# AzureLeon1/DiffSpectra

Hardware: AMD Instinct MI355X
Metric: molecules/sec, 1000-step QM9S all-spectra sampling (partial run) (higher is better)
Workload: dtype f32 (GEMMs as split-fp16 x3 MFMA with fp32 accumulate; fp32-level accuracy, parity gates unchanged)

## Files before the change

### diffspectra_amd/csrc/ds_kernels.hip

```cpp
#include <hip/hip_runtime.h>
#include <math.h>
#include <stdint.h>
#include <stdio.h>
#include <stdlib.h>

#include <atomic>
#include <mutex>
#include <utility>
#include <vector>

#include "../../include/diffspectra_hip.h"
#include "ds_device.h"
#include "ds_train_common.h"

#define ADAC DS_ADA_COLS
constexpr int DS_NODE_PF = 8;
constexpr int DS_NODE_PF2 = 4;
constexpr int DS_QKV_PF = 4;
constexpr int DS_TWO_STREAM_MAX_PAIRS = 400000;

#ifdef DS_STAMPS
#define DS_STAMP_INIT()                                                                                 \
  unsigned long long _sa[16] = {0, 0, 0, 0, 0, 0, 0, 0, 0, 0, 0, 0, 0, 0, 0, 0};                        \
  unsigned long long _t0 = __builtin_amdgcn_s_memtime()
#define DS_STAMP(i)                                                                                     \
  do {                                                                                                  \
    const unsigned long long _t1 = __builtin_amdgcn_s_memtime();                                        \
    _sa[i] += _t1 - _t0;                                                                                \
    _t0 = _t1;                                                                                          \
  } while (0)
#define DS_STAMP_W(i)                                                                                   \
  do {                                                                                                  \
    asm volatile("s_waitcnt vmcnt(0) lgkmcnt(0)" ::: "memory");                                         \
    DS_STAMP(i);                                                                                        \
  } while (0)
#define DS_STAMP_FLUSH(t)                                                                               \
  do {                                                                                                  \
    if (threadIdx.x == (t))                                                                             \
      for (int _i = 0; _i < 16; ++_i)                                                                   \
        if (_sa[_i]) atomicAdd(reinterpret_cast<unsigned long long*>(c.ws.flags + 16) + _i, _sa[_i]);   \
  } while (0)
#else
#define DS_STAMP_INIT()
#define DS_STAMP(i)
#define DS_STAMP_W(i)
#define DS_STAMP_FLUSH(t)
#endif

namespace {

struct Ctx {
  ds_layout L;
  ds_workspace ws;
  const float* wbase;
  const int64_t* woff;
  float edge_th, cutoff;
};

__device__ __forceinline__ const float* BW(const Ctx& c, int blk, int slot) {
  return c.wbase + c.woff[blk * DS_W_BLOCK_SLOTS + slot];
}
__device__ __forceinline__ const float* GW(const Ctx& c, int slot) {
  return c.wbase + c.woff[DS_NBLOCKS * DS_W_BLOCK_SLOTS + slot];
}

__device__ __forceinline__ float rbf_feature(float x, int k, const float* __restrict__ mean, const float* __restrict__ stdv,
                                             const float* __restrict__ astd) {
  if (k == 0) return x;
  const float z = (x - mean[k - 1]) / stdv[k - 1];
  return expf(-0.5f * (z * z)) / astd[k - 1];
}

__global__ void k_time_feat(Ctx c, const float* __restrict__ noise_level) {
  const int b = blockIdx.x * blockDim.x + threadIdx.x;
  if (b >= c.L.B) return;
  const float* w = GW(c, DS_GW_SIN_W);
  const float x = noise_level[b];
  float* f = c.ws.tfeat + (size_t)b * 24;
  f[0] = x;
  for (int i = 0; i < 8; ++i) {
    const float fr = ((x * w[i]) * 2.0f) * 3.14159265358979323846f;
    f[1 + i] = sinf(fr);
    f[9 + i] = cosf(fr);
  }
  for (int i = 17; i < 24; ++i) f[i] = 0.0f;
}

__global__ void k_pair_flags(Ctx c, const float* __restrict__ cond_x, const float* __restrict__ cond_edge_x) {
  const int p = blockIdx.x * blockDim.x + threadIdx.x;
  const bool valid = p < c.L.Pp;
  int bits = 3;
  bool nonzero = false;
  if (valid && cond_x != nullptr) {
    const int da = c.L.node_dense[c.L.pair_a[p]], db = c.L.node_dense[c.L.pair_b[p]];
    const float* pa = cond_x + (size_t)da * 9;
    const float* pb = cond_x + (size_t)db * 9;
    const float dx = pa[0] - pb[0], dy = pa[1] - pb[1], dz = pa[2] - pb[2];
    const float d2 = dx * dx + dy * dy + dz * dz;
    const int m = c.L.pair_mol[p];
    const int lb = db - m * c.L.N;
    const float ce = cond_edge_x[((size_t)da * c.L.N + lb) * 2 + 0];
    bits = (ce >= c.edge_th ? 1 : 0) | (d2 <= c.cutoff ? 2 : 0);
    nonzero = d2 != 0.0f;
  }
  if (valid) c.ws.adj[p] = bits;
  if (cond_x != nullptr) {
    const int any = __syncthreads_or(nonzero ? 1 : 0);
    if (any && threadIdx.x == 0) __hip_atomic_store(&c.ws.flags[0], 1, __ATOMIC_RELAXED, __HIP_MEMORY_SCOPE_AGENT);
  }
}

__global__ __launch_bounds__(256) void k_node_init(Ctx c, const float* __restrict__ xh, const float* __restrict__ cond_x) {
  constexpr int R = 8;
  const int row0 = blockIdx.x * R;
  const int col = threadIdx.x;
  __shared__ __attribute__((aligned(16))) float in[R][16];
  if (col < R * 16) {
    const int rr = col >> 4, k = col & 15, row = row0 + rr;
    float v = 0.0f;
    if (row < c.L.Nn) {
      const int d = c.L.node_dense[row];
      if (k < 6) v = xh[(size_t)d * 9 + 3 + k];
      else if (k < 12) v = cond_x ? cond_x[(size_t)d * 9 + 3 + (k - 6)] : 0.0f;
      else if (k < 15) v = xh[(size_t)d * 9 + (k - 12)];
    }
    in[rr][k] = v;
  }
  __syncthreads();
  const float* W = GW(c, DS_GW_NODE_EMB_W);
  float w[12];
#pragma unroll
  for (int k = 0; k < 12; ++k) w[k] = wp_at(W, 256, k, col);
  const float bias = GW(c, DS_GW_NODE_EMB_B)[col];
#pragma unroll
  for (int rr = 0; rr < R; ++rr) {
    const int row = row0 + rr;
    if (row >= c.L.Nn) break;
    float acc = 0.0f;
#pragma unroll
// ... 132 lines not shown
    for (int i = 0; i < 16; ++i) acc[0][i] = bcol;
    acc_zero<1>(lo);
    wave_mma_h_deep<1, false, 8, 8>(&Xh[mt * 32][0], 128, wse, ring, 0, acc, lo);
    split_finish<1>(acc, lo);
#pragma unroll
    for (int i = 0; i < 16; ++i) Y[mt * 32 + acc_row(i, lane >> 5)][cc * 32 + (lane & 31)] = acc[0][i];
  }
  __syncthreads();
  {
    const int lane = tid & 63, wv = tid >> 6;
    _Float16* ye = reinterpret_cast<_Float16*>(c.ws.ye);
#pragma unroll
    for (int j = 0; j < 4; ++j) {
      const int row = 16 * wv + 4 * j + (lane >> 4);
      const float4 v = ln_mod_reg64(reinterpret_cast<const float4*>(&Y[row][0])[lane & 15], lsh[j], lsc[j]);
      if (row0 + row < c.L.Pp) split_store4(ye + (size_t)(row0 + row) * 128, 64, 4 * (lane & 15), v);
    }
  }
}

template <int NW>
__global__ __launch_bounds__(NW * 64) void k_node_qkv(Ctx c, int blk) {
  ds_fp16_saturate();
  constexpr int NT = NW * 64;
  constexpr int T = 64;
  constexpr int LDH = 2 * 256 + 8;
  __shared__ __attribute__((aligned(16))) _Float16 Xh[T][LDH];
  __shared__ int rmol[T];
  const int tid = threadIdx.x, row0 = blockIdx.x * T, col0 = blockIdx.y * 384;
  if (tid < T) rmol[tid] = (row0 + tid < c.L.Nn) ? c.L.node_mol[row0 + tid] : 0;
  __syncthreads();
  {
    const float* adn = c.ws.ada + blk * DS_ADA_BLOCK_STRIDE + DS_ADA_NODE;
    const int lane = tid & 63, wv = tid >> 6, g = lane >> 4, j = lane & 15;
    static_assert(NT == 256, "four waves x 16 rows");
#pragma unroll
    for (int half = 0; half < 2; ++half) {
      float4 v[2][4], sh[2][4], sc[2][4];
#pragma unroll
      for (int ps = 0; ps < 2; ++ps) {
        const int row = 16 * wv + 8 * half + 4 * ps + g;
        const float4* hp = reinterpret_cast<const float4*>(c.ws.h + (size_t)min(row0 + row, c.L.Nn - 1) * 256) + j;
        const float4* ap = reinterpret_cast<const float4*>(adn + (size_t)rmol[row] * ADAC) + j;
#pragma unroll
        for (int u = 0; u < 4; ++u) {
          v[ps][u] = hp[16 * u];
          sh[ps][u] = ap[16 * u];
          sc[ps][u] = ap[64 + 16 * u];
        }
      }
#pragma unroll
      for (int ps = 0; ps < 2; ++ps) {
        const int row = 16 * wv + 8 * half + 4 * ps + g;
        ln_mod_quad256(v[ps], sh[ps], sc[ps]);
#pragma unroll
        for (int u = 0; u < 4; ++u)
          split_store4(&Xh[row][0], 256, 64 * u + 4 * j, row0 + row < c.L.Nn ? v[ps][u] : make_float4(0, 0, 0, 0));
      }
    }
  }
  __syncthreads();
  const float* bias = BW(c, blk, DS_BW_QKV_B) + col0;
  float* qkv = c.ws.qkv + (size_t)row0 * 768 + col0;
  const int valid = c.L.Nn - row0, wave = tid >> 6;
  for (int ch = wave; ch < 12; ch += NW) {
    asm volatile("" ::: "memory");
    const float b = bias[ch * 32 + (tid & 31)];
    f32x16 acc[2], lo[2];
#pragma unroll
    for (int m = 0; m < 2; ++m)
#pragma unroll
      for (int i = 0; i < 16; ++i) acc[m][i] = b;
    acc_zero<2>(lo);
    wave_mma_h_ring<2, false, 16, DS_QKV_PF>(&Xh[0][0], 256, BW(c, blk, DS_BW_QKV_H), 768, 256, col0 + ch * 32, 0, acc, lo);
    split_finish<2>(acc, lo);
    acc_store<2, 768>(acc, qkv + ch * 32, valid, [](int, float v) { return v; });
  }
}

__global__ __launch_bounds__(1024) void k_attn_fused(Ctx c, int blk) {
  ds_fp16_saturate();
  DS_STAMP_INIT();
  constexpr int NT = 1024, QS = 512 + 32, LDT = 256 + 4, LDY = 2 * 64 + 8, CR = 32, MAXP = DS_MAX_ATOMS * (DS_MAX_ATOMS - 1) / 2;
  __shared__ __attribute__((aligned(16))) float QK[DS_MAX_ATOMS * QS];
  __shared__ __attribute__((aligned(16))) float Tt[2][CR][LDT];
  __shared__ __attribute__((aligned(16))) _Float16 Yc[2][CR][LDY];
  __shared__ __attribute__((aligned(16))) float AL[2][CR][32];
  __shared__ int PT[(MAXP + 15) & ~15];
  __shared__ int VT[32][32];
  static_assert(DS_MAX_ATOMS <= 32 && MAXP <= 511 - CR, "visit table packing");
  static_assert(DS_MAX_ATOMS * 128 <= 4 * NT && DS_MAX_ATOMS * 64 <= 2 * NT && MAXP <= NT, "single-pass staging");
  const int tid = threadIdx.x, wave = tid >> 6, lane = tid & 63, hh = lane >> 5;
  int n0, n, p0, P;
  if (c.L.mol_by_size) {
    const int4 r = reinterpret_cast<const int4*>(c.L.mol_by_size)[blockIdx.x];
    n0 = r.x; n = r.y; p0 = r.z; P = r.w;
  } else {
    const int m = blockIdx.x;
    n0 = c.L.node_off[m]; n = c.L.node_off[m + 1] - n0;
    p0 = c.L.pair_off[m]; P = c.L.pair_off[m + 1] - p0;
  }
  const WStreamH ws_e0 = wstream_h(BW(c, blk, DS_BW_E0_H), 256, 64, (wave & 7) * 32);
  const WStreamH ws_e1 = wstream_h(BW(c, blk, DS_BW_E1_H), 256, 64, (wave & 7) * 32);
  if (n <= 0) return;
  if (P <= 0) {
    for (int i = tid; i < 256; i += NT) c.ws.attn[(size_t)n0 * 256 + i] = 0.0f;
    return;
  }
  const int nch = (P + CR - 1) / CR;
  const bool producer = wave >= 8;
  const int ptid = tid & 511, prow = ptid >> 4, ppiece = ptid & 15;
  const u32x4* ye4 = reinterpret_cast<const u32x4*>(c.ws.ye) + (size_t)p0 * 16;
  auto row_pair = [&](int R) {
    const int d = R / n + 1, i = R - (d - 1) * n;
    int j = i + d;
    if (j >= n) j -= n;
    const int a = min(i, j), b = max(i, j);
    return a * (2 * n - a - 1) / 2 + (b - a - 1);
  };
  auto fetch_y = [&](int ck, bool class_order) {
    const int R = ck * CR + prow;
    const int Rc = min(R, P - 1);
    return ye4[(size_t)(class_order ? PT[Rc] : Rc) * 16 + ppiece];
  };
  auto commit_y = [&](int buf, const u32x4& v) { *reinterpret_cast<u32x4*>(&Yc[buf][prow][ppiece * 8]) = v; };
  h8 wf[2][4];
  auto load_weights = [&](const WStreamH& ws_) {
#pragma unroll
    for (int pl = 0; pl < 2; ++pl)
#pragma unroll
      for (int kb = 0; kb < 4; ++kb) wf[pl][kb] = wload_h(ws_, pl, kb);
  };
  auto project = [&](int buf) {
    f32x16 acc[1], lo[1];
    acc_zero<1>(acc);
    acc_zero<1>(lo);
    const _Float16* xr = &Yc[buf][lane & 31][8 * hh];
#pragma unroll
    for (int kb = 0; kb < 4; ++kb) {
      const h8 x1 = *reinterpret_cast<const h8*>(xr + kb * 16);
      const h8 x2 = *reinterpret_cast<const h8*>(xr + 64 + kb * 16);
      acc[0] = __builtin_amdgcn_mfma_f32_32x32x16_f16(wf[0][kb], x1, acc[0], 0, 0, 0);
      lo[0] = __builtin_amdgcn_mfma_f32_32x32x16_f16(wf[0][kb], x2, lo[0], 0, 0, 0);
      lo[0] = __builtin_amdgcn_mfma_f32_32x32x16_f16(wf[1][kb], x1, lo[0], 0, 0, 0);
    }
    split_finish<1>(acc, lo);
    float* trow = &Tt[buf][lane & 31][(wave & 7) * 32 + 4 * hh];
#pragma unroll
    for (int q = 0; q < 4; ++q) {
      f32x2 v0, v1;
      v0.x = acc[0][4 * q]; v0.y = acc[0][4 * q + 1]; v1.x = acc[0][4 * q + 2]; v1.y = acc[0][4 * q + 3];
      v0 = ds_tanh2_prescaled(v0); v1 = ds_tanh2_prescaled(v1);
      *reinterpret_cast<float4*>(trow + 8 * q) = make_float4(v0.x, v0.y, v1.x, v1.y);
    }
  };
  auto produce = [&](u32x4 ya, u32x4 yb, bool class_order, auto&& after_first) {
    project(0);
    after_first();
    if (1 < nch) commit_y(1, ya);
    if (3 < nch) ya = fetch_y(3, class_order);
    __syncthreads();
    if (class_order) { DS_STAMP(13); } else { DS_STAMP(9); }
    auto interval = [&](int k, u32x4& B) {
      if (k + 2 < nch) commit_y(k & 1, B);
      if (k + 4 < nch) B = fetch_y(k + 4, class_order);
      if (k + 1 < nch) project((k + 1) & 1);
      if (class_order) { DS_STAMP(14); } else { DS_STAMP(10); }
      __syncthreads();
      if (class_order) { DS_STAMP(15); } else { DS_STAMP(11); }
    };
    for (int k = 0; k < nch; k += 2) {
      interval(k, yb);
      if (k + 1 >= nch) break;
      interval(k + 1, ya);
    }
  };

  {
    u32x4 y0 = {0, 0, 0, 0}, y1 = y0, y2 = y0;
    if (producer) {
      load_weights(ws_e0);
      y0 = fetch_y(0, false);
      y1 = fetch_y(1, false);
      y2 = fetch_y(2, false);
    } else if (tid < P) {
      PT[tid] = ((c.L.pair_a[p0 + tid] - n0) << 8) | (c.L.pair_b[p0 + tid] - n0) | (c.ws.adj[p0 + tid] << 16);
    }
    f32x4 v[4];
#pragma unroll
    for (int u = 0; u < 4; ++u) {
      const int idx = min(tid + u * NT, n * 128 - 1);
      v[u] = reinterpret_cast<const f32x4*>(c.ws.qkv + (size_t)(n0 + (idx >> 7)) * 768)[idx & 127];
    }
    __builtin_amdgcn_sched_barrier(0);
    auto store_qk = [&]() {
      f32x4* junk = reinterpret_cast<f32x4*>(&Tt[1][0][0]) + tid;
#pragma unroll
      for (int u = 0; u < 4; ++u) {
        const int idx = tid + u * NT;
        f32x4* dst = idx < n * 128 ? reinterpret_cast<f32x4*>(QK) + (idx >> 7) * (QS / 4) + (idx & 127) : junk;
        *dst = v[u];
      }
    };
    if (producer) commit_y(0, y0);
    __syncthreads();
    if (producer) { DS_STAMP(8); } else { DS_STAMP(0); }
    if (producer) {
      produce(y1, y2, false, store_qk);
      load_weights(ws_e1);
    } else {
      store_qk();
      __syncthreads();
      DS_STAMP(1);
      const int row = tid >> 4, hs = tid & 15;
      for (int k = 0; k < nch; ++k) {
        const int pl = k * CR + row;
        if (pl < P) {
          const int e_ = PT[pl];
          float* out = c.ws.lg + (size_t)(p0 + pl) * 32;
          if (hs == 14) {
            const float h0 = (e_ & 0x10000) ? 1.0f : -1e10f, h1 = (e_ & 0x20000) ? 1.0f : -1e10f;
            out[0] = h0; out[1] = h1; out[16] = h0; out[17] = h1;
          } else if (hs < 14) {
            const int a = (e_ >> 8) & 255, b = e_ & 255;
            typedef const volatile f32x2 __attribute__((address_space(3))) * lds_v2;
            lds_v2 t0 = (lds_v2)(&Tt[k & 1][row][hs * 18]);
            lds_v2 qa = (lds_v2)(QK + a * QS + hs * 18);
            lds_v2 qb = (lds_v2)(QK + b * QS + hs * 18);
            lds_v2 ka = (lds_v2)(QK + a * QS + 256 + hs * 18);
            lds_v2 kb = (lds_v2)(QK + b * QS + 256 + hs * 18);
            float s_ab = 0.0f, s_ba = 0.0f;
#pragma unroll
            for (int j0 = 0; j0 < 9; j0 += 3) {
              f32x2 e[3], xa[3], xb[3], ya[3], yb[3];
#pragma unroll
              for (int j = 0; j < 3; ++j) { e[j] = t0[j0 + j]; xa[j] = qa[j0 + j]; xb[j] = qb[j0 + j]; ya[j] = ka[j0 + j]; yb[j] = kb[j0 + j]; }
#pragma unroll
              for (int j = 0; j < 3; ++j) {
                s_ab = __builtin_fmaf(xb[j].x * ya[j].x, e[j].x, s_ab); s_ab = __builtin_fmaf(xb[j].y * ya[j].y, e[j].y, s_ab);
                s_ba = __builtin_fmaf(xa[j].x * yb[j].x, e[j].x, s_ba); s_ba = __builtin_fmaf(xa[j].y * yb[j].y, e[j].y, s_ba);
              }
            }
            out[2 + hs] = s_ab / 4.0f;
            out[16 + 2 + hs] = s_ba / 4.0f;
          }
        }
        DS_STAMP(2);
        __syncthreads();
        DS_STAMP(3);
      }
    }
  }
  __threadfence_block();
  __syncthreads();
  float* V = QK;
  int* ET = reinterpret_cast<int*>(&Tt[0][0][0]);
  {
    const int t = tid >> 5, q = tid & 31, d = (q >> 1) + 1;
    int e = 511;
    if (t < n && q < n - 1) {
      int i, s_;
      if (2 * d == n) {
        i = t < d ? t : t - d;
        s_ = t < d ? t + d : t - d;
      } else {
        int sa = t + d, ib = t - d;
        if (sa >= n) sa -= n;
        if (ib < 0) ib += n;
        const bool first_is_a = t < ib;
        const bool take_a = (q & 1) ? !first_is_a : first_is_a;
        i = take_a ? t : ib;
        s_ = take_a ? sa : ib;
      }
      e = ((d - 1) * n + i) | (s_ << 9) | ((s_ < t ? 0 : 1) << 14);
    }
    VT[t][q] = e;
    const int s = q;
    int eo = -1;
    if (t < n && s < n && s != t) {
      const int lo_ = s < t ? s : t, hi_ = s < t ? t : s;
      eo = (lo_ * (2 * n - lo_ - 1) / 2 + (hi_ - lo_ - 1)) * 32 + (s < t ? 0 : 16);
    }
    ET[t * 32 + s] = eo;
    if (tid < P) PT[tid] = row_pair(tid);
  }
  f32x4 vst[2];
#pragma unroll
  for (int u = 0; u < 2; ++u) {
    const int i0 = min(tid + u * NT, n * 64 - 1);
    vst[u] = reinterpret_cast<const f32x4*>(c.ws.qkv + (size_t)(n0 + (i0 >> 6)) * 768 + 512)[i0 & 63];
  }
  __builtin_amdgcn_sched_barrier(0);
  __syncthreads();
  u32x4 y0 = {0, 0, 0, 0}, y1 = y0, y2 = y0;
  if (producer) {
    y0 = fetch_y(0, true);
    y1 = fetch_y(1, true);
    y2 = fetch_y(2, true);
  }
  auto store_v = [&]() {
    f32x4* junk = reinterpret_cast<f32x4*>(&Yc[0][0][0]) + tid;
#pragma unroll
    for (int u = 0; u < 2; ++u) {
      f32x4* dst = tid + u * NT < n * 64 ? reinterpret_cast<f32x4*>(V) + tid + u * NT : junk;
      *dst = vst[u];
    }
  };
  {
    const int h = lane & 15, sq = (lane >> 4) & 1, t = 2 * wave + hh;
    const int* et = ET + t * 32 + sq;
    float* lgm = c.ws.lg + (size_t)p0 * 32 + h;
    if (t < n) {
      float x[15];
      int eos[15];
      float mx = -INFINITY;
#pragma unroll
      for (int j = 0; j < 15; ++j) eos[j] = et[2 * j];
#pragma unroll
      for (int j = 0; j < 15; ++j) x[j] = lgm[max(eos[j], 0)];
      __builtin_amdgcn_sched_barrier(0);
#pragma unroll
      for (int j = 0; j < 15; ++j) x[j] = eos[j] >= 0 ? x[j] : -INFINITY;
#pragma unroll
      for (int j = 0; j < 15; ++j) mx = fmaxf(mx, x[j]);
      mx = fmaxf(mx, __shfl_xor(mx, 16, 64));
      float sum = 0.0f;
#pragma unroll
      for (int j = 0; j < 15; ++j) {
        x[j] = __expf(x[j] - mx);
        sum += x[j];
      }
      sum += __shfl_xor(sum, 16, 64);
      const float den = sum + 1e-16f;
#pragma unroll
      for (int j = 0; j < 15; ++j)
        if (eos[j] >= 0) lgm[eos[j]] = x[j] / den;
    }
  }
  store_v();
  __threadfence_block();
  __syncthreads();
  if (producer) { DS_STAMP(12); } else { DS_STAMP(4); }
  if (producer) {
    commit_y(0, y0);
    __syncthreads();
    produce(y1, y2, true, [] {});
    DS_STAMP_FLUSH(512);
  } else {
    const int arow = (tid & 255) >> 3, apiece = tid & 7;
    auto fetch_a = [&](int ck) {
      const int R = ck * CR + arow;
      return reinterpret_cast<const u32x4*>(c.ws.lg + (size_t)(p0 + PT[min(R, P - 1)]) * 32)[apiece];
    };
    auto commit_a = [&](int buf, const u32x4& v) {
      if (tid < 256) reinterpret_cast<u32x4*>(&AL[buf][arow][0])[apiece] = v;
    };
    const u32x4 a0 = fetch_a(0);
    u32x4 ab = fetch_a(1), aa = fetch_a(2);
    commit_a(0, a0);
    __syncthreads();
    __syncthreads();
    DS_STAMP(5);
    const int t_me = tid >> 4, q16 = tid & 15;
    const int* vt_row = &VT[t_me][0];
    int vt_q = 0, vt_e = vt_row[0];
    float4 acc[4];
#pragma unroll
    for (int u = 0; u < 4; ++u) acc[u] = make_float4(0, 0, 0, 0);
    auto interval = [&](int k, u32x4& A) {
      if (k + 1 < nch) commit_a((k + 1) & 1, A);
      if (k + 3 < nch) A = fetch_a(k + 3);
      const int R0 = k * CR;
      while ((vt_e & 511) - R0 < CR) {
        const int r = (vt_e & 511) - R0, s_ = (vt_e >> 9) & 31;
        const float4* gp = reinterpret_cast<const float4*>(&Tt[k & 1][r][4 * q16]);
        const float4* vp = reinterpret_cast<const float4*>(V + s_ * 256 + 4 * q16);
        const float* ap = &AL[k & 1][r][((vt_e >> 14) & 1) * 16 + (q16 >> 2)];
        float4 g[4], v[4];
        float al[4];
#pragma unroll
        for (int u = 0; u < 4; ++u) { g[u] = gp[16 * u]; v[u] = vp[16 * u]; al[u] = ap[4 * u]; }
        vt_e = vt_row[++vt_q];
#pragma unroll
        for (int u = 0; u < 4; ++u) {
          acc[u].x += (v[u].x * g[u].x) * al[u]; acc[u].y += (v[u].y * g[u].y) * al[u];
          acc[u].z += (v[u].z * g[u].z) * al[u]; acc[u].w += (v[u].w * g[u].w) * al[u];
        }
      }
      DS_STAMP(6);
      __syncthreads();
      DS_STAMP(7);
    };
    for (int k = 0; k < nch; k += 2) {
      interval(k, ab);
      if (k + 1 >= nch) break;
      interval(k + 1, aa);
    }
    if (t_me < n) {
      float4* o = reinterpret_cast<float4*>(c.ws.attn + (size_t)(n0 + t_me) * 256 + 4 * q16);
#pragma unroll
      for (int u = 0; u < 4; ++u) o[16 * u] = acc[u];
    }
    DS_STAMP_FLUSH(0);
  }
}

__global__ __launch_bounds__(256) void k_node_n2e(Ctx c, int blk) {
  ds_fp16_saturate();
  constexpr int T = 64, LDH = 2 * 256 + 8;
  __shared__ __attribute__((aligned(16))) _Float16 A1[T][LDH];
  const int tid = threadIdx.x, wave = tid >> 6, lane = tid & 63, row0 = blockIdx.x * T;
  const int Nn = c.L.Nn;
  {
    float4 v[16];
#pragma unroll
    for (int u = 0; u < 16; ++u) {
      const int idx = tid + u * 256, row = idx >> 6, k4 = idx & 63;
      v[u] = reinterpret_cast<const float4*>(c.ws.attn + (size_t)min(row0 + row, Nn - 1) * 256)[k4];
    }
#pragma unroll
    for (int u = 0; u < 16; ++u) {
      const int idx = tid + u * 256, row = idx >> 6, k4 = idx & 63;
      split_store4(&A1[row][0], 256, 4 * k4, row0 + row < Nn ? v[u] : make_float4(0, 0, 0, 0));
    }
  }
  __syncthreads();
  const int mt = wave >> 1, cc = wave & 1;
  if (row0 + mt * 32 >= Nn) return;
  f32x16 acc[1], lo[1];
  acc_zero<1>(acc);
  acc_zero<1>(lo);
  wave_mma_h_ring<1, false, 16, DS_NODE_PF>(&A1[mt * 32][0], 256, BW(c, blk, DS_BW_N2E_H), 64, 256, cc * 32, 0, acc, lo);
  split_finish<1>(acc, lo);
  acc_store<1, 64>(acc, c.ws.u + (size_t)(row0 + mt * 32) * 64 + cc * 32, Nn - row0 - mt * 32, [](int, float v) { return v; });
  (void)lane;
}

template <bool N2E>
__global__ __launch_bounds__(256, 2) void k_node_update(Ctx c, int blk) {
  ds_fp16_saturate();
  constexpr int T = 32, LDH = 2 * 256 + 8;
  __shared__ __attribute__((aligned(16))) _Float16 B1[T][LDH];
  __shared__ __attribute__((aligned(16))) _Float16 H2[T][LDH];
  __shared__ int rmol[T];
  const int tid = threadIdx.x, wave = tid >> 6, row0 = blockIdx.x * T;
  const int Nn = c.L.Nn;
  const float* ada = c.ws.ada;
  if (tid < T) rmol[tid] = (row0 + tid < Nn) ? c.L.node_mol[row0 + tid] : 0;
  __syncthreads();
  {
    const int lane = tid & 63, g = lane >> 4, j = lane & 15;
    float4 va[2][4], vh[2][4], vg[2][4], sh[2][4], sc[2][4];
#pragma unroll
    for (int ps = 0; ps < 2; ++ps) {
      const int row = 8 * wave + 4 * ps + g;
      const size_t gr = (size_t)min(row0 + row, Nn - 1);
      const float4* ad = reinterpret_cast<const float4*>(ada + (size_t)rmol[row] * ADAC + blk * DS_ADA_BLOCK_STRIDE + DS_ADA_NODE) + j;
      const float4* ap = reinterpret_cast<const float4*>(c.ws.attn + gr * 256) + j;
      const float4* hp = reinterpret_cast<const float4*>(c.ws.h + gr * 256) + j;
#pragma unroll
      for (int u = 0; u < 4; ++u) {
        va[ps][u] = ap[16 * u];
        vh[ps][u] = hp[16 * u];
        vg[ps][u] = ad[128 + 16 * u];
        sh[ps][u] = ad[192 + 16 * u];
        sc[ps][u] = ad[256 + 16 * u];
      }
    }
#pragma unroll
    for (int ps = 0; ps < 2; ++ps) {
      const int row = 8 * wave + 4 * ps + g;
      float4 r[4];
#pragma unroll
      for (int u = 0; u < 4; ++u) {
        if (row0 + row >= Nn) va[ps][u] = vh[ps][u] = make_float4(0, 0, 0, 0);
        if (N2E) split_store4(&B1[row][0], 256, 64 * u + 4 * j, va[ps][u]);
        r[u].x = vh[ps][u].x + vg[ps][u].x * va[ps][u].x; r[u].y = vh[ps][u].y + vg[ps][u].y * va[ps][u].y;
        r[u].z = vh[ps][u].z + vg[ps][u].z * va[ps][u].z; r[u].w = vh[ps][u].w + vg[ps][u].w * va[ps][u].w;
      }
      ln_mod_quad256(r, sh[ps], sc[ps]);
#pragma unroll
      for (int u = 0; u < 4; ++u) split_store4(&H2[row][0], 256, 64 * u + 4 * j, r[u]);
    }
  }
  __syncthreads();
  if (N2E) {
    if (wave < 2) {
// ... 1168 lines not shown
        if (c_bond2[ta][tb] != 0 && d < (float)(c_bond2[ta][tb] + 5)) {
          order = 2;
          if (c_bond3[ta][tb] != 0 && d < (float)(c_bond3[ta][tb] + 3)) order = 3;
        }
      }
      bonds += order;
      if (bond_order) bond_order[(size_t)dn[a] * N + (dn[b] - m * N)] = order;
    }
    ok = bonds == c_valence[ta] ? 1 : 0;
  }
  const int cnt = __popcll(__ballot(ok != 0));
  if (a == 0) { nr_stable[m] = cnt; mol_stable[m] = cnt == n ? 1 : 0; }
}

__global__ __launch_bounds__(1024) void k_spec_attention(const float* __restrict__ qkv, float* __restrict__ scores,
                                                       float* __restrict__ out, int B, int L, int heads, float scale,
                                                       int has_prev) {
  constexpr int DK = 8;
  extern __shared__ __attribute__((aligned(16))) float kv[];
  const int b = blockIdx.z, h = blockIdx.y, q0 = blockIdx.x * blockDim.x, tid = threadIdx.x;
  const int D = heads * DK;
  float* Ks = kv;
  float* Vs = kv + (size_t)L * DK;
  for (int idx = tid; idx < L * DK; idx += blockDim.x) {
    const int j = idx / DK, d = idx - j * DK;
    const float* base = qkv + ((size_t)b * L + j) * 3 * D + h * DK + d;
    Ks[idx] = base[D];
    Vs[idx] = base[2 * D];
  }
  __syncthreads();
  const int i = q0 + tid;
  if (i >= L) return;
  float q[DK];
  for (int d = 0; d < DK; ++d) q[d] = qkv[((size_t)b * L + i) * 3 * D + h * DK + d];
  float* scol = scores + ((size_t)b * heads + h) * L * L + i;
  float mx = -INFINITY, den = 0.0f, o[DK];
  for (int d = 0; d < DK; ++d) o[d] = 0.0f;
  for (int j0 = 0; j0 < L; j0 += 8) {
    float sv[8];
    float bm = -INFINITY;
#pragma unroll
    for (int u = 0; u < 8; ++u) {
      const int j = min(j0 + u, L - 1);
      float s = 0.0f;
#pragma unroll
      for (int d = 0; d < DK; ++d) s += q[d] * Ks[j * DK + d];
      s *= scale;
      if (has_prev) s += scol[(size_t)j * L];
      sv[u] = s;
      if (j0 + u < L) { scol[(size_t)j * L] = s; bm = fmaxf(bm, s); }
    }
    const float nm = fmaxf(mx, bm), r = expf(mx - nm);
    den *= r;
#pragma unroll
    for (int d = 0; d < DK; ++d) o[d] *= r;
#pragma unroll
    for (int u = 0; u < 8; ++u) {
      if (j0 + u < L) {
        const float p = expf(sv[u] - nm);
        den += p;
#pragma unroll
        for (int d = 0; d < DK; ++d) o[d] += p * Vs[(j0 + u) * DK + d];
      }
    }
    mx = nm;
  }
  for (int d = 0; d < DK; ++d) out[((size_t)b * L + i) * D + h * DK + d] = o[d] / den;
}

__global__ void k_layernorm_affine(const float* __restrict__ x, const float* __restrict__ g, const float* __restrict__ bt,
                                   float* __restrict__ y, int rows, int cols, float eps) {
  const int row = blockIdx.x, lane = threadIdx.x;
  if (row >= rows) return;
  const float* xr = x + (size_t)row * cols;
  float s = 0.0f;
  for (int k = lane; k < cols; k += 64) s += xr[k];
  const float mean = wave_sum(s) / (float)cols;
  float v = 0.0f;
  for (int k = lane; k < cols; k += 64) { const float d = xr[k] - mean; v += d * d; }
  const float rstd = 1.0f / sqrtf(wave_sum(v) / (float)cols + eps);
  for (int k = lane; k < cols; k += 64) y[(size_t)row * cols + k] = (xr[k] - mean) * rstd * g[k] + bt[k];
}

bool make_ctx(Ctx& c, const ds_weights* w, const ds_layout* L, const ds_workspace* ws) {
  if (!w || !L || !ws || !w->base || !w->off_dev) return false;
  if (L->max_n > DS_MAX_ATOMS || L->B <= 0) return false;
  c.L = *L; c.ws = *ws; c.wbase = w->base; c.woff = w->off_dev;
  c.edge_th = w->edge_th; c.cutoff = w->spatial_cut_off;
  return true;
}

inline bool layout_ok(const ds_layout* L) { return L && L->B > 0 && L->max_n <= DS_MAX_ATOMS && L->max_n <= L->N; }

inline bool clear(void* p, size_t bytes, hipStream_t s) { return hipMemsetAsync(p, 0, bytes, s) == hipSuccess; }
inline bool record(hipEvent_t ev, hipStream_t s) { return hipEventRecord(ev, s) == hipSuccess; }
inline bool wait(hipStream_t s, hipEvent_t ev) { return hipStreamWaitEvent(s, ev, 0) == hipSuccess; }
constexpr int MAX_DEVICES = 16;

inline int device_cus() {
  static std::atomic<int> cus[MAX_DEVICES];
  int dev = 0, n = 0;
  if (hipGetDevice(&dev) != hipSuccess || dev < 0 || dev >= MAX_DEVICES) return 256;
  if ((n = cus[dev].load(std::memory_order_relaxed)) > 0) return n;
  if (hipDeviceGetAttribute(&n, hipDeviceAttributeMultiprocessorCount, dev) != hipSuccess || n <= 0) n = 256;
  cus[dev].store(n, std::memory_order_relaxed);
  return n;
}

template <int ACT>
__global__ __launch_bounds__(256, 2) void k_gemm_big(GemmArgs g) {
  constexpr int T = 128, KC = 64, LD = KC + DS_LDP;
  __shared__ __attribute__((aligned(16))) float X[2][T][LD];
  const int tid = threadIdx.x, wave = tid >> 6;
  const int row0 = blockIdx.x * T;
  const int col0 = (blockIdx.y * 4 + wave) * 32;
  const bool active = col0 < g.Npad;
  const int nchunks = g.K / KC;
  float4 st[8];
  auto fetch = [&](int kc) {
#pragma unroll
    for (int u = 0; u < 8; ++u) {
      const int idx = tid + u * 256, row = idx >> 4, k4 = idx & 15;
      const size_t gr = (size_t)min(row0 + row, g.M - 1);
      st[u] = reinterpret_cast<const float4*>(g.A + gr * g.lda + (size_t)kc * KC)[k4];
    }
  };
  auto stash = [&](int buf) {
#pragma unroll
    for (int u = 0; u < 8; ++u) {
      const int idx = tid + u * 256, row = idx >> 4, k4 = idx & 15;
      float4 v = st[u];
      if (g.a_silu) { v.x = ds_silu(v.x); v.y = ds_silu(v.y); v.z = ds_silu(v.z); v.w = ds_silu(v.w); }
      if (row0 + row >= g.M) v = make_float4(0, 0, 0, 0);
      reinterpret_cast<float4*>(&X[buf][row][0])[k4] = v;
    }
  };
  f32x16 acc[4];
  acc_zero<4>(acc);
  fetch(0);
  stash(0);
  BFrag bf = bfrag_load(g.Wp, g.Npad, active ? col0 : 0, 0, 8);
  __syncthreads();
  for (int kc = 0; kc < nchunks; ++kc) {
    const int cur = kc & 1;
    if (kc + 1 < nchunks) fetch(kc + 1);
    const float* wp = g.Wp + (size_t)(kc * (KC / 8)) * 2 * g.Npad * 4;
    if (active) wave_mma<4>(&X[cur][0][0], LD, wp, g.Npad, col0, 0, KC / 8, acc, 0, &bf);
    if (kc + 1 < nchunks) {
      stash(cur ^ 1);
      bf = bfrag_load(wp + (size_t)(KC / 8) * 2 * g.Npad * 4, g.Npad, active ? col0 : 0, 0, 8);
    }
    __syncthreads();
  }
  if (!active) return;
  {
    const int lane = tid & 63, r = lane & 31, hh = lane >> 5, col = col0 + r;
    const bool colok = col < g.N;
    const float bcol = (g.bias && colok) ? g.bias[col] : 0.0f;
    const float csc = (g.cs && colok) ? g.cs[col] : 1.0f, csh = (g.cs && colok) ? g.csh[col] : 0.0f;
    const unsigned long long pw = reinterpret_cast<unsigned long long>(g.C + (size_t)row0 * g.ldc + col0);
    const unsigned long long pu = (static_cast<unsigned long long>(__builtin_amdgcn_readfirstlane(static_cast<int>(pw >> 32))) << 32) |
                                  static_cast<unsigned int>(__builtin_amdgcn_readfirstlane(static_cast<int>(pw)));
    const __amdgpu_buffer_rsrc_t rc = __builtin_amdgcn_make_buffer_rsrc(reinterpret_cast<float*>(pu), 0, 0x7fffffff, 0x00020000);
    const int voff = (4 * hh * g.ldc + r) * 4, rowb = g.ldc * 4;
#pragma unroll
    for (int m = 0; m < 4; ++m)
#pragma unroll
      for (int i = 0; i < 16; ++i) {
        const int row = m * 32 + (i & 3) + 8 * (i >> 2), gr = row0 + row + 4 * hh;
        if (gr < g.M && colok) {
          float v = ds_act<ACT>(acc[m][i] + bcol);
// ... 137 lines not shown
  Ctx c;
  if (!make_ctx(c, w, L, ws) || !xh || !edge_x || ((cond_x == nullptr) != (cond_edge_x == nullptr))) return DS_ERR_ARG;
  if (!clear(ws->flags, 8 * sizeof(int32_t), s)) return DS_ERR_LAUNCH;
  if (L->Pp > 0) hipLaunchKernelGGL(k_pair_flags, dim3((L->Pp + 1023) / 1024), dim3(1024), 0, s, c, cond_x, cond_edge_x);
  hipLaunchKernelGGL(k_node_init, dim3((L->Nn + 7) / 8), dim3(256), 0, s, c, xh, cond_x);
  if (L->Pp > 0) hipLaunchKernelGGL(k_pair_init, dim3((L->Pp + 63) / 64), dim3(256), 0, s, c, edge_x, cond_x, cond_edge_x);
  return DST_CHECK_LAUNCH();
}

int ds_stage_block(const ds_weights* w, const ds_layout* L, ds_workspace* ws, int blk, int last, void* stream) {
  hipStream_t s = (hipStream_t)stream;
  Ctx c;
  if (!make_ctx(c, w, L, ws) || blk < 0 || blk >= DS_NBLOCKS) return DS_ERR_ARG;
  launch_edge_geom(c, blk, s);
  launch_node_qkv(c, blk, s);
  launch_attn(c, blk, s);
  launch_node_update<true>(c, blk, s);
  launch_edge_update(c, blk, s);
  launch_equi_pairs(c, blk, s);
  launch_pos_update(c, last, s);
  return DST_CHECK_LAUNCH();
}

int ds_stage_readout(const ds_weights* w, const ds_layout* L, ds_workspace* ws, float* out_xh, float* out_edge, void* stream) {
  hipStream_t s = (hipStream_t)stream;
  Ctx c;
  if (!make_ctx(c, w, L, ws) || !out_xh || !out_edge) return DS_ERR_ARG;
  const size_t nx = (size_t)L->B * L->N * 9, ne = (size_t)L->B * L->N * L->N * 2;
  if (!clear(out_xh, nx * sizeof(float), s) || !clear(out_edge, ne * sizeof(float), s)) return DS_ERR_LAUNCH;
  hipLaunchKernelGGL(k_node_readout, dim3((L->Nn + 31) / 32), dim3(256), 0, s, c, out_xh);
  if (L->Pp > 0) hipLaunchKernelGGL(k_edge_readout, dim3((L->Pp + 127) / 128), dim3(256), 0, s, c, out_edge);
  hipLaunchKernelGGL(k_final_pos, dim3((L->B + 63) / 64), dim3(64), 0, s, c, out_xh);
  return DST_CHECK_LAUNCH();
}

struct SideStream {
  hipStream_t s = nullptr;
  hipEvent_t fork[DS_NBLOCKS + 1] = {}, join[DS_NBLOCKS + 1] = {};
  std::once_flag once;
  bool ok = false;
};
static SideStream g_side[MAX_DEVICES];
static int g_two_stream = -1;

static SideStream* side_stream() {
  int dev = 0;
  if (hipGetDevice(&dev) != hipSuccess || dev < 0 || dev >= MAX_DEVICES) return nullptr;
  SideStream& ss = g_side[dev];
  std::call_once(ss.once, [&ss] {
    bool ok = hipStreamCreateWithFlags(&ss.s, hipStreamNonBlocking) == hipSuccess;
    for (int i = 0; ok && i <= DS_NBLOCKS; ++i)
      ok = hipEventCreateWithFlags(&ss.fork[i], hipEventDisableTiming) == hipSuccess &&
           hipEventCreateWithFlags(&ss.join[i], hipEventDisableTiming) == hipSuccess;
    ss.ok = ok;
  });
  return ss.ok ? &ss : nullptr;
}

static int forward_blocks_two_streams(const ds_weights* w, const ds_layout* L, ds_workspace* ws, hipStream_t s, SideStream* ss) {
  Ctx c;
  if (!make_ctx(c, w, L, ws)) return DS_ERR_ARG;
  hipStream_t s2 = ss->s;
  const hipEvent_t fork0 = ss->fork[DS_NBLOCKS], join0 = ss->join[DS_NBLOCKS];
  if (!record(fork0, s) || !wait(s2, fork0)) return DS_ERR_LAUNCH;
  launch_node_qkv(c, 0, s2);
  if (!record(join0, s2)) return DS_ERR_LAUNCH;
  for (int blk = 0; blk < DS_NBLOCKS; ++blk) {
    launch_edge_geom(c, blk, s);
    if (!wait(s, blk == 0 ? join0 : ss->join[blk - 1])) return DS_ERR_LAUNCH;
    launch_attn(c, blk, s);
    launch_node_n2e(c, blk, s);
    if (!record(ss->fork[blk], s) || !wait(s2, ss->fork[blk])) return DS_ERR_LAUNCH;
    launch_node_update<false>(c, blk, s2);
    if (blk + 1 < DS_NBLOCKS) launch_node_qkv(c, blk + 1, s2);
    if (!record(ss->join[blk], s2)) return DS_ERR_LAUNCH;
    launch_edge_update(c, blk, s);
    if (!wait(s, ss->join[blk])) return DS_ERR_LAUNCH;
    launch_equi_pairs(c, blk, s);
    launch_pos_update(c, blk == DS_NBLOCKS - 1 ? 1 : 0, s);
  }
  return DST_CHECK_LAUNCH();
}

int ds_set_two_stream(int on) {
  const int prev = g_two_stream;
  g_two_stream = on;
  return prev;
}

int ds_forward(const ds_weights* w, const ds_layout* L, ds_workspace* ws, const float* xh, const float* edge_x,
               const float* cond_x, const float* cond_edge_x, const float* noise_level, const float* ctx_emb, float* out_xh,
               float* out_edge, void* stream) {
  int st = ds_stage_time(w, L, ws, noise_level, ctx_emb, stream);
  if (st) return st;
  st = ds_stage_init(w, L, ws, xh, edge_x, cond_x, cond_edge_x, stream);
  if (st) return st;
  static const int env_two = [] { const char* e = getenv("DIFFSPECTRA_TWO_STREAM"); return e ? atoi(e) : -1; }();
  const int pick = g_two_stream >= 0 ? g_two_stream : env_two;
  const int two = pick >= 0 ? pick : (L->Pp < DS_TWO_STREAM_MAX_PAIRS ? 1 : 0);
  SideStream* ss = two ? side_stream() : nullptr;
  if (ss) {
    st = forward_blocks_two_streams(w, L, ws, (hipStream_t)stream, ss);
    if (st) return st;
  } else {
    for (int b = 0; b < DS_NBLOCKS; ++b) {
      st = ds_stage_block(w, L, ws, b, b == DS_NBLOCKS - 1, stream);
      if (st) return st;
    }
  }
  return ds_stage_readout(w, L, ws, out_xh, out_edge, stream);
}

int ds_sampler_step(const ds_layout* L, float c_x, float c_pred, float sigma, float temperature, float* x, float* edge_x,
                     const float* pred, const float* edge_pred, const float* raw_pos, const float* raw_feat,
                     const float* raw_edge, float* x_mean, float* edge_mean, void* stream) {
  if (!layout_ok(L) || !x || !edge_x || !pred || !edge_pred || !raw_pos || !raw_feat || !raw_edge || !x_mean || !edge_mean) return DS_ERR_ARG;
  hipLaunchKernelGGL(k_sampler_step, dim3(L->B), dim3(256), 0, (hipStream_t)stream, *L, c_x, c_pred, sigma, temperature, x,
                     edge_x, pred, edge_pred, raw_pos, raw_feat, raw_edge, x_mean, edge_mean);
  return DST_CHECK_LAUNCH();
}

int ds_initial_noise(const ds_layout* L, uint64_t seed, const int64_t* mol_id, float* x, float* edge_x, void* stream) {
  if (!layout_ok(L) || !mol_id || !x || !edge_x) return DS_ERR_ARG;
  hipStream_t s = (hipStream_t)stream;
  const size_t nb = (size_t)L->B * L->N;
  if (!clear(x, nb * 9 * sizeof(float), s) || !clear(edge_x, nb * L->N * 2 * sizeof(float), s)) return DS_ERR_LAUNCH;
  hipLaunchKernelGGL(k_noise_step<0>, dim3(L->B), dim3(256), 0, s, *L, 0.0f, 0.0f, 0.0f, 0.0f, (unsigned long long)seed, 0u, mol_id,
                     x, edge_x, (const float*)nullptr, (const float*)nullptr, (float*)nullptr, (float*)nullptr,
                     (const float*)nullptr, (const int32_t*)nullptr);
  return DST_CHECK_LAUNCH();
}

int ds_sampler_step_philox(const ds_layout* L, float c_x, float c_pred, float sigma, float temperature, uint64_t seed, int32_t step,
                           const int64_t* mol_id, float* x, float* edge_x, const float* pred, const float* edge_pred,
                           float* x_mean, float* edge_mean, void* stream) {
  if (!layout_ok(L) || !mol_id || !x || !edge_x || !pred || !edge_pred || !x_mean || !edge_mean || step < 0) return DS_ERR_ARG;
  hipLaunchKernelGGL(k_noise_step<1>, dim3(L->B), dim3(256), 0, (hipStream_t)stream, *L, c_x, c_pred, sigma, temperature,
                     (unsigned long long)seed, (unsigned int)step + 1u, mol_id, x, edge_x, pred, edge_pred, x_mean, edge_mean,
                     (const float*)nullptr, (const int32_t*)nullptr);
  return DST_CHECK_LAUNCH();
}

int ds_step_begin(const float* table, int32_t n_steps, int32_t* step, int32_t B, float* noise_level, void* stream) {
  if (!table || !step || !noise_level || B <= 0 || n_steps <= 0) return DS_ERR_ARG;
  hipLaunchKernelGGL(k_step_begin, dim3(1), dim3(256), 0, (hipStream_t)stream, table, n_steps, step, B, noise_level);
  return DST_CHECK_LAUNCH();
}

int ds_sampler_step_philox_dev(const ds_layout* L, const float* table, const int32_t* step, float temperature, uint64_t seed,
                               const int64_t* mol_id, float* x, float* edge_x, const float* pred, const float* edge_pred,
                               float* x_mean, float* edge_mean, void* stream) {
  if (!layout_ok(L) || !table || !step || !mol_id || !x || !edge_x || !pred || !edge_pred || !x_mean || !edge_mean) return DS_ERR_ARG;
  hipLaunchKernelGGL(k_noise_step<2>, dim3(L->B), dim3(256), 0, (hipStream_t)stream, *L, 0.0f, 0.0f, 0.0f, temperature,
                     (unsigned long long)seed, 0u, mol_id, x, edge_x, pred, edge_pred, x_mean, edge_mean, table, step);
  return DST_CHECK_LAUNCH();
}

int ds_post_process(const ds_layout* L, const float* xh, const float* edge_x, float* pos_out, int32_t* atom_type, int32_t* fc,
                    float* edge_type, void* stream) {
  if (!layout_ok(L) || !xh || !edge_x || !pos_out || !atom_type || !fc || !edge_type) return DS_ERR_ARG;
  hipStream_t s = (hipStream_t)stream;
  const size_t nb = (size_t)L->B * L->N;
  if (!clear(pos_out, nb * 3 * sizeof(float), s) || !clear(atom_type, nb * sizeof(int32_t), s) || !clear(fc, nb * sizeof(int32_t), s) ||
      !clear(edge_type, nb * L->N * sizeof(float), s))
    return DS_ERR_LAUNCH;
  hipLaunchKernelGGL(k_post_process, dim3(L->B), dim3(128), 0, s, *L, xh, edge_x, pos_out, atom_type, fc, edge_type);
// ... 58 lines not shown
```

### include/diffspectra_hip.h

```cpp
#ifndef DIFFSPECTRA_HIP_H
#define DIFFSPECTRA_HIP_H

#include <stdint.h>

#ifdef __cplusplus
extern "C" {
#endif

#define DS_OK 0
#define DS_ERR_ARG (-1)
#define DS_ERR_LAUNCH (-2)

#define DS_NBLOCKS 8
#define DS_HID 256
#define DS_EHID 64
#define DS_TDIM 1024
#define DS_ADA_BLOCK_STRIDE 2464
#define DS_ADA_NODE 0
#define DS_ADA_EDGE 1536
#define DS_ADA_EQUI 1920
#define DS_ADA_DIST 2432
#define DS_ADA_TOP (DS_NBLOCKS * DS_ADA_BLOCK_STRIDE)
#define DS_ADA_COLS (DS_ADA_TOP + 32)

// ... 40 lines not shown
};
#define DS_W_NUM_SLOTS (DS_NBLOCKS * DS_W_BLOCK_SLOTS + DS_W_GLOBAL_SLOTS)

#define DS_MAX_ATOMS 29
#define DS_RECORD_BYTES 1248
#define DS_REC_POS 0
#define DS_REC_TYPE (DS_MAX_ATOMS * 12)
#define DS_REC_FC (DS_REC_TYPE + DS_MAX_ATOMS)
#define DS_REC_BOND (DS_REC_FC + DS_MAX_ATOMS)
#define DS_REC_BOND_END (DS_REC_BOND + DS_MAX_ATOMS * DS_MAX_ATOMS)
#ifdef __cplusplus
static_assert(DS_REC_BOND_END <= DS_RECORD_BYTES && DS_RECORD_BYTES % 4 == 0, "a record holds its fields and is a whole number of dwords");
static_assert((DS_REC_BOND_END + 3) / 4 * 4 <= DS_RECORD_BYTES, "the dwords that cover the bond block stay inside the record");
#endif


typedef struct ds_weights {
  const float* base;
  const int64_t* off_dev;
  int64_t off[DS_W_NUM_SLOTS];
  float edge_th;
  float spatial_cut_off;
} ds_weights;

typedef struct ds_layout {
  int32_t B, N, Nn, Pp;
  int32_t max_n;
  int32_t _pad;
  const int32_t* node_off;
  const int32_t* pair_off;
  const int32_t* node_dense;
  const int32_t* node_mol;
  const int32_t* pair_a;
  const int32_t* pair_b;
  const int32_t* pair_mol;
  const int32_t* mol_by_size;
} ds_layout;

typedef struct ds_workspace {
  float* pos;
  float* h;
  float* e;
  float* atom_hids;
  float* edge_hids;
  float* tfeat;
  float* tmid;
  float* temb_silu;
  float* ada;
  float* qkv;
  float* ye;
  float* dist;
  float* attn;
  float* u;
  float* ac;
  float* ed;
  float* lg;
  float* tr;
  int32_t* adj;
  int32_t* flags;
} ds_workspace;

void ds_struct_sizes(int64_t* out);

typedef struct ds_gemm_args {
  const float* A; int64_t lda; int32_t a_grp_rows; int32_t _p0; int64_t a_grp_stride;
  const float* Wp; const float* bias;
  float* C; int64_t ldc; int32_t c_grp_rows; int32_t _p1; int64_t c_grp_stride;
  int32_t M, K, N, act;
  const float* R; int64_t ldr; int32_t r_grp_rows; int32_t a_silu;
  const float* col_scale; const float* col_shift;
} ds_gemm_args;
int ds_gemm(const ds_gemm_args* args, void* stream);

int ds_gemm_split(const void* A_split, const float* W_split, const float* bias, float* C, int64_t ldc, int32_t M, int32_t K,
                  int32_t N, void* stream);

int ds_forward(const ds_weights* w, const ds_layout* L, ds_workspace* ws,
               const float* xh, const float* edge_x, const float* cond_x, const float* cond_edge_x,
               const float* noise_level, const float* ctx_emb,
               float* out_xh, float* out_edge, void* stream);

int ds_set_two_stream(int on);

int ds_stage_time(const ds_weights* w, const ds_layout* L, ds_workspace* ws, const float* noise_level,
                  const float* ctx_emb, void* stream);
int ds_stage_init(const ds_weights* w, const ds_layout* L, ds_workspace* ws, const float* xh, const float* edge_x,
                  const float* cond_x, const float* cond_edge_x, void* stream);
int ds_stage_block(const ds_weights* w, const ds_layout* L, ds_workspace* ws, int block, int last, void* stream);
int ds_stage_readout(const ds_weights* w, const ds_layout* L, ds_workspace* ws, float* out_xh, float* out_edge,
                     void* stream);

int ds_sampler_step(const ds_layout* L, float c_x, float c_pred, float sigma, float temperature,
                    float* x, float* edge_x, const float* pred, const float* edge_pred,
                    const float* raw_pos, const float* raw_feat, const float* raw_edge,
                    float* x_mean, float* edge_mean, void* stream);

int ds_initial_noise(const ds_layout* L, uint64_t seed, const int64_t* mol_id, float* x, float* edge_x, void* stream);
int ds_sampler_step_philox(const ds_layout* L, float c_x, float c_pred, float sigma, float temperature,
                           uint64_t seed, int32_t step, const int64_t* mol_id,
                           float* x, float* edge_x, const float* pred, const float* edge_pred,
                           float* x_mean, float* edge_mean, void* stream);

int ds_step_begin(const float* table, int32_t n_steps, int32_t* step, int32_t B, float* noise_level, void* stream);
int ds_sampler_step_philox_dev(const ds_layout* L, const float* table, const int32_t* step, float temperature,
                               uint64_t seed, const int64_t* mol_id, float* x, float* edge_x, const float* pred,
                               const float* edge_pred, float* x_mean, float* edge_mean, void* stream);

int ds_post_process(const ds_layout* L, const float* xh, const float* edge_x,
                    float* pos_out, int32_t* atom_type, int32_t* fc, float* edge_type, void* stream);

int ds_check_stability(const ds_layout* L, const float* pos, const int32_t* atom_type, int32_t* bond_order,
                       int32_t* nr_stable, int32_t* mol_stable, void* stream);

int ds_match_records(const uint8_t* prb_rec, const int32_t* prb_n, int64_t P, const uint8_t* ref_rec, const int32_t* ref_n, int64_t M,
                     const int64_t* ref_index, float max_distance, int32_t min_atoms, double* rmsd, int32_t* n_matched,
                     float* type_acc, float* bond_acc, uint8_t* exact, int32_t* map, void* stream);

#define DS_GRAPH_DIFFERENT 0
#define DS_GRAPH_IDENTICAL 1
#define DS_GRAPH_UNDECIDED 2
#define DS_GRAPH_INVALID 3
#define DS_GRAPH_MAX_NODES 1048576
int ds_graph_identity_records(const uint8_t* prb_rec, const int32_t* prb_n, int64_t P, const uint8_t* ref_rec, const int32_t* ref_n, int64_t M,
                              const int64_t* ref_index, int32_t max_nodes, uint8_t* verdict, int32_t* nodes, int32_t* map, void* stream);

int ds_graph_hash_records(const uint8_t* rec, const int32_t* n, int64_t P, uint64_t* hash, void* stream);

#define DS_MCES_EXACT 0
#define DS_MCES_UNDECIDED 2
#define DS_MCES_INVALID 3
#define DS_MCES_MAX_NODES 4194304
int ds_mces_records(const uint8_t* prb_rec, const int32_t* prb_n, int64_t P, const uint8_t* ref_rec, const int32_t* ref_n, int64_t M,
                    const int64_t* ref_index, int32_t drop_h, int32_t max_nodes, int32_t* dist, int32_t* lower, uint8_t* status,
                    int32_t* nodes, int32_t* map, void* stream);

#define DS_MORGAN_MAX_RADIUS 3
#define DS_MORGAN_MAX_FEATURES 116
#define DS_MORGAN_MAX_BITS 4096
#define DS_MORGAN_OK 0
#define DS_MORGAN_INVALID 3
int ds_morgan_records(const uint8_t* rec, const int32_t* n, int64_t P, int32_t drop_h, int32_t radius, uint64_t* ids, int32_t* count,
                      void* stream);
int ds_morgan_similarity_records(const uint8_t* prb_rec, const int32_t* prb_n, int64_t P, const uint8_t* ref_rec, const int32_t* ref_n, int64_t M,
                                 const int64_t* ref_index, int32_t drop_h, int32_t radius, int32_t n_bits, int32_t* common, int32_t* n_prb,
                                 int32_t* n_ref, uint8_t* status, void* stream);

#define DS_GEOM_MAX_CLASSES 32
int ds_geometry_count_records(const uint8_t* rec, const int32_t* n, int64_t P, const int32_t* bond_cls, int32_t n_bond_cls,
                              const int32_t* angle_cls, int32_t n_angle_cls, const int32_t* dihedral_cls, int32_t n_dihedral_cls,
                              int32_t* counts, int32_t* skipped, void* stream);
int ds_geometry_fill_records(const uint8_t* rec, const int32_t* n, int64_t P, const int32_t* bond_cls, int32_t n_bond_cls,
                             const int32_t* angle_cls, int32_t n_angle_cls, const int32_t* dihedral_cls, int32_t n_dihedral_cls,
                             int64_t total_bond, int64_t total_angle, int64_t total_dihedral, const int64_t* offsets,
                             float* bond_value, uint8_t* bond_class, float* angle_value, uint8_t* angle_class,
                             float* dihedral_value, uint8_t* dihedral_class, void* stream);

#define DS_MMD_TILE 256
#define DS_MMD_CHUNKS 128
#define DS_MMD_MAX_SAMPLES 1048576
#define DS_MMD_MAX_KERNELS 8
#define DS_MMD_MAX_CLASSES 65535
#define DS_MMD_OK 0
#define DS_MMD_EMPTY 1
#define DS_MMD_INVALID 2
int ds_mmd_1d_workspace_bytes(int64_t n_classes, int64_t* bytes);
int ds_mmd_1d_segments(const float* x, const int64_t* x_off, int64_t Nx, const float* y, const int64_t* y_off, int64_t Ny, int64_t n_classes,
// ... 18 lines not shown
```

Before: 232.5.

## Keep attention logits and weights in LDS arena instead of global round-trip

The fused attention kernel now carves a single LDS arena of about 160KB. When a molecule's q|k tile and per-pair logits fit, the logits and softmax weights stay in shared memory instead of round-tripping through the global lg buffer. That removes the global fetch/commit pipeline for alpha tiles and the block-scope fences. The visit table gains a packed pair index so the aggregation step can read alpha from LDS directly, and global lg is still written for later consumers. The larger LDS footprint may reduce occupancy, and there is an env/API toggle.

```diff
diff --git a/diffspectra_amd/csrc/ds_kernels.hip b/diffspectra_amd/csrc/ds_kernels.hip
--- a/diffspectra_amd/csrc/ds_kernels.hip
+++ b/diffspectra_amd/csrc/ds_kernels.hip
@@ -6,6 +6,7 @@
 
 #include <atomic>
 #include <mutex>
+#include <type_traits>
 #include <utility>
 #include <vector>
 
@@ -55,6 +56,7 @@
   const float* wbase;
   const int64_t* woff;
   float edge_th, cutoff;
+  int attn_lds;
 };
 
 __device__ __forceinline__ const float* BW(const Ctx& c, int blk, int slot) {
@@ -353,13 +355,15 @@
   ds_fp16_saturate();
   DS_STAMP_INIT();
   constexpr int NT = 1024, QS = 512 + 32, LDT = 256 + 4, LDY = 2 * 64 + 8, CR = 32, MAXP = DS_MAX_ATOMS * (DS_MAX_ATOMS - 1) / 2;
-  __shared__ __attribute__((aligned(16))) float QK[DS_MAX_ATOMS * QS];
   __shared__ __attribute__((aligned(16))) float Tt[2][CR][LDT];
   __shared__ __attribute__((aligned(16))) _Float16 Yc[2][CR][LDY];
-  __shared__ __attribute__((aligned(16))) float AL[2][CR][32];
   __shared__ int PT[(MAXP + 15) & ~15];
   __shared__ int VT[32][32];
-  static_assert(DS_MAX_ATOMS <= 32 && MAXP <= 511 - CR, "visit table packing");
+  constexpr int QK_F = DS_MAX_ATOMS * QS, AL_F = 2 * CR * 32;
+  constexpr int ARENA_F = (160 * 1024 - (int)(sizeof(Tt) + sizeof(Yc) + sizeof(PT) + sizeof(VT))) / 4 & ~3;
+  __shared__ __attribute__((aligned(16))) float ARENA[ARENA_F];
+  static_assert(QK_F + AL_F <= ARENA_F && QK_F % 4 == 0, "the global path's q|k and alpha tiles");
+  static_assert(DS_MAX_ATOMS <= 32 && MAXP <= 511 - CR && MAXP <= (1 << 16), "visit table packing: row 9 bits, source 5, direction 1, pair row 16");
   static_assert(DS_MAX_ATOMS * 128 <= 4 * NT && DS_MAX_ATOMS * 64 <= 2 * NT && MAXP <= NT, "single-pass staging");
   const int tid = threadIdx.x, wave = tid >> 6, lane = tid & 63, hh = lane >> 5;
   int n0, n, p0, P;
@@ -378,6 +382,12 @@
     for (int i = tid; i < 256; i += NT) c.ws.attn[(size_t)n0 * 256 + i] = 0.0f;
     return;
   }
+  const bool lds_lg = c.attn_lds && n * QS + P * 32 <= ARENA_F;
+  float* const QK = ARENA;
+  float (*const AL)[CR][32] = reinterpret_cast<float (*)[CR][32]>(ARENA + QK_F);
+  float* const LG = ARENA + ARENA_F - P * 32;
+  auto body = [&](auto lds_tag) {
+  constexpr bool LDS_LG = decltype(lds_tag)::value;
   const int nch = (P + CR - 1) / CR;
   const bool producer = wave >= 8;
   const int ptid = tid & 511, prow = ptid >> 4, ppiece = ptid & 15;
@@ -488,7 +498,7 @@
         const int pl = k * CR + row;
         if (pl < P) {
           const int e_ = PT[pl];
-          float* out = c.ws.lg + (size_t)(p0 + pl) * 32;
+          float* out = LDS_LG ? LG + pl * 32 : c.ws.lg + (size_t)(p0 + pl) * 32;
           if (hs == 14) {
             const float h0 = (e_ & 0x10000) ? 1.0f : -1e10f, h1 = (e_ & 0x20000) ? 1.0f : -1e10f;
             out[0] = h0; out[1] = h1; out[16] = h0; out[17] = h1;
@@ -522,7 +532,7 @@
       }
     }
   }
-  __threadfence_block();
+  if constexpr (!LDS_LG) __threadfence_block();
   __syncthreads();
   float* V = QK;
   int* ET = reinterpret_cast<int*>(&Tt[0][0][0]);
@@ -544,6 +554,10 @@
         s_ = take_a ? sa : ib;
       }
       e = ((d - 1) * n + i) | (s_ << 9) | ((s_ < t ? 0 : 1) << 14);
+      if constexpr (LDS_LG) {
+        const int lo_ = min(s_, t), hi_ = max(s_, t);
+        e |= (lo_ * (2 * n - lo_ - 1) / 2 + (hi_ - lo_ - 1)) << 15;
+      }
     }
     VT[t][q] = e;
     const int s = q;
@@ -580,7 +594,8 @@
   {
     const int h = lane & 15, sq = (lane >> 4) & 1, t = 2 * wave + hh;
     const int* et = ET + t * 32 + sq;
-    float* lgm = c.ws.lg + (size_t)p0 * 32 + h;
+    float* glg = c.ws.lg + (size_t)p0 * 32 + h;
+    float* lgm = LDS_LG ? LG + h : glg;
     if (t < n) {
       float x[15];
       int eos[15];
@@ -605,11 +620,15 @@
       const float den = sum + 1e-16f;
 #pragma unroll
       for (int j = 0; j < 15; ++j)
-        if (eos[j] >= 0) lgm[eos[j]] = x[j] / den;
+        if (eos[j] >= 0) {
+          const float a = x[j] / den;
+          lgm[eos[j]] = a;
+          if constexpr (LDS_LG) glg[eos[j]] = a;
+        }
     }
   }
   store_v();
-  __threadfence_block();
+  if constexpr (!LDS_LG) __threadfence_block();
   __syncthreads();
   if (producer) { DS_STAMP(12); } else { DS_STAMP(4); }
   if (producer) {
@@ -626,9 +645,12 @@
     auto commit_a = [&](int buf, const u32x4& v) {
       if (tid < 256) reinterpret_cast<u32x4*>(&AL[buf][arow][0])[apiece] = v;
     };
-    const u32x4 a0 = fetch_a(0);
-    u32x4 ab = fetch_a(1), aa = fetch_a(2);
-    commit_a(0, a0);
+    u32x4 ab = {0, 0, 0, 0}, aa = ab;
+    if constexpr (!LDS_LG) {
+      const u32x4 a0 = fetch_a(0);
+      ab = fetch_a(1); aa = fetch_a(2);
+      commit_a(0, a0);
+    }
     __syncthreads();
     __syncthreads();
     DS_STAMP(5);
@@ -639,14 +661,17 @@
 #pragma unroll
     for (int u = 0; u < 4; ++u) acc[u] = make_float4(0, 0, 0, 0);
     auto interval = [&](int k, u32x4& A) {
-      if (k + 1 < nch) commit_a((k + 1) & 1, A);
-      if (k + 3 < nch) A = fetch_a(k + 3);
+      if constexpr (!LDS_LG) {
+        if (k + 1 < nch) commit_a((k + 1) & 1, A);
+        if (k + 3 < nch) A = fetch_a(k + 3);
+      }
       const int R0 = k * CR;
       while ((vt_e & 511) - R0 < CR) {
         const int r = (vt_e & 511) - R0, s_ = (vt_e >> 9) & 31;
         const float4* gp = reinterpret_cast<const float4*>(&Tt[k & 1][r][4 * q16]);
         const float4* vp = reinterpret_cast<const float4*>(V + s_ * 256 + 4 * q16);
-        const float* ap = &AL[k & 1][r][((vt_e >> 14) & 1) * 16 + (q16 >> 2)];
+        const float* ap = LDS_LG ? LG + (vt_e >> 15) * 32 + ((vt_e >> 14) & 1) * 16 + (q16 >> 2)
+                                 : &AL[k & 1][r][((vt_e >> 14) & 1) * 16 + (q16 >> 2)];
         float4 g[4], v[4];
         float al[4];
 #pragma unroll
@@ -674,6 +699,9 @@
     }
     DS_STAMP_FLUSH(0);
   }
+  };
+  if (lds_lg) body(std::true_type{});
+  else body(std::false_type{});
 }
 
 __global__ __launch_bounds__(256) void k_node_n2e(Ctx c, int blk) {
@@ -2008,11 +2036,13 @@
   for (int k = lane; k < cols; k += 64) y[(size_t)row * cols + k] = (xr[k] - mean) * rstd * g[k] + bt[k];
 }
 
+std::atomic<int> g_attn_lds{-1};
 bool make_ctx(Ctx& c, const ds_weights* w, const ds_layout* L, const ds_workspace* ws) {
   if (!w || !L || !ws || !w->base || !w->off_dev) return false;
   if (L->max_n > DS_MAX_ATOMS || L->B <= 0) return false;
   c.L = *L; c.ws = *ws; c.wbase = w->base; c.woff = w->off_dev;
   c.edge_th = w->edge_th; c.cutoff = w->spatial_cut_off;
+  c.attn_lds = g_attn_lds != 0;
   return true;
 }
 
@@ -2316,6 +2346,10 @@
   return DST_CHECK_LAUNCH();
 }
 
+int ds_set_attn_lds(int on) {
+  return g_attn_lds.exchange(on < 0 ? -1 : on != 0);
+}
+
 int ds_set_two_stream(int on) {
   const int prev = g_two_stream;
   g_two_stream = on;
diff --git a/include/diffspectra_hip.h b/include/diffspectra_hip.h
--- a/include/diffspectra_hip.h
+++ b/include/diffspectra_hip.h
@@ -146,6 +146,8 @@
 
 int ds_set_two_stream(int on);
 
+int ds_set_attn_lds(int on);
+
 int ds_stage_time(const ds_weights* w, const ds_layout* L, ds_workspace* ws, const float* noise_level,
                   const float* ctx_emb, void* stream);
 int ds_stage_init(const ds_weights* w, const ds_layout* L, ds_workspace* ws, const float* xh, const float* edge_x,
```

Result: no change. 233.2, median of 6 (+0.3%).
